# sloup/hessgpu

Hardware: AMD Instinct MI355X
Metric: Mpixels/s end-to-end (pyramid->descriptor), 1920x1080 (higher is better)
Workload: dtype f32; 1 GPU; 1920x1080 synthetic blobs (tests/fixtures.py), default octaves/DoG levels, top-K=4096 [configs[1]]; pipelined_contexts_per_gpu=6, streams_and_copier_threads_per_node=6, descriptor_order=pixel, distinct_images_per_gpu=8, input=u8 luminance resident in HBM; results delivered to host memory

## Files before the change

hessgpu_amd/csrc/hess_ctx.h:

```cpp
#pragma once
#include <hip/hip_runtime.h>
#include <hsa/hsa.h>
#include <hsa/hsa_ext_amd.h>

#include <algorithm>
#include <atomic>
#include <cmath>
#include <condition_variable>
#include <cstdarg>
#include <cerrno>
#include <chrono>
#include <cstdio>
#include <cstdlib>
#include <cstring>
#include <mutex>
#include <new>
#include <string>
#include <thread>
#include <vector>

#include <fcntl.h>
#include <limits.h>
#include <sys/mman.h>
#include <sys/stat.h>
// ... 112 lines not shown
  int ds = 0;
  int img_w = 0, img_h = 0;
  Geom g;
  Taps taps0;
  bool has_taps0 = false;
  int cap_raw = 0, cap_sel = 0, cap_feat = 0;
  bool use_topk = false, multi = false;
  int dim = 0;
  int found_tasks = 0;
  DevBuf gauss, deth, got, input_f32, upsampled, stage, rowoff, level_count, raw_total, found, task_count, raw, sel,
      sel_total, recs, ocount, foffset, fsrc, feat_total, feat_first, img_base, keys, desc;
  DevBuf zeroed;
  size_t zeroed_used = 0;
  bool zero_filled = false;
  struct View { void* p = nullptr; } rowmask, rowcnt, overflow, hist, tk,
      found_count, place_ticket, place_flag;
  int batch = 0;
  int pyramid_batch = 0;
  std::vector<int> counts;
  std::vector<size_t> offs;
  DevBuf h_keys, h_desc, h_small;
  std::string share;
  struct ShareDir {
    uint32_t magic, gen_keys, gen_desc, pad;
    uint64_t keys_bytes, desc_bytes;
    char keys_path[1024], desc_path[1024];
  }* share_dir = nullptr;
  bool share_by_need = false;
  DevBuf h_stage;
  double stamp_submit0 = 0.0, stamp_submit1 = 0.0;
  bool level0_in_lds = false;
// ... 102 lines not shown
```

hessgpu_amd/csrc/hess_dev.h:

```cpp
#pragma once
#include <hip/hip_runtime.h>
#include <stdint.h>

namespace hess {

constexpr int kMaxOct = 16;
constexpr int kMaxDog = 10;
constexpr int kMaxLev = kMaxDog + 3;
constexpr int kMaxTaps = 33;
#ifndef HESS_STREAM_NC
#define HESS_STREAM_NC 2
#endif
constexpr int kStreamCols = HESS_STREAM_NC;
constexpr int kStreamPitch = 62 * kStreamCols;
#ifndef HESS_STREAM_ROWS
#define HESS_STREAM_ROWS 24
#endif
constexpr int kStreamRows = HESS_STREAM_ROWS;
constexpr int kHistBins = 32768;

typedef float hess_v4f __attribute__((ext_vector_type(4)));
__device__ __forceinline__ void store_stream_f4(float* p, float x, float y, float z, float w) {
#ifdef HESS_NO_STREAM_STORES
  *reinterpret_cast<float4*>(p) = make_float4(x, y, z, w);
#else
  __builtin_nontemporal_store((hess_v4f){x, y, z, w}, reinterpret_cast<hess_v4f*>(p));
#endif
}

// ... 151 lines not shown
void launch_dog_planes(hipStream_t st, const Geom& g, const float* gauss, float* deth, int level_max, int batch);
void launch_hessian_level(hipStream_t st, const Geom& g, const float* gauss, float* deth, int level, float norm,
                          int batch, void* zero = nullptr, size_t zero_bytes = 0);

constexpr int kDetectSlots = 64;
struct DetectStore {
  RawKey* found;
  long long stride;
  int ntask;
  int* task_count;
  int* spill_count;
  int cap_spill;
  unsigned* hist;
};
int extrema_tasks(const Geom& g);
void launch_extrema_mark(hipStream_t st, const Geom& g, const DetectParams& dp, const float* gauss,
                         const float* deth, uint64_t* rowmask, int* rowcnt, const DetectStore& ds, int batch,
                         bool dog_mode = false);
bool extrema_streams(const Geom& g);
void launch_extrema_place(hipStream_t st, const Geom& g, const LimitParams& lp, const DetectStore& ds, const uint64_t* rowmask,
                          const int* rowcnt, int* rowoff, int* level_count, int* raw_total, int* overflow, int* ticket,
                          int* flag, RawKey* raw, int cap_raw, int batch);

void launch_topk(hipStream_t st, const Geom& g, int K, const RawKey* raw, const int* raw_total,
                 int cap_raw, unsigned* hist, RawKey* sel, int* sel_total, int cap_sel, int batch, void* scratch,
                 int* overflow);
size_t topk_scratch_bytes(int cap_raw, int batch, int nlev);

void launch_orientation(hipStream_t st, const Geom& g, const OrientParams& op, const RawKey* list,
                        const int* list_total, int cap_list, const float* got, FRec* recs,
                        int* ocount, int batch);
void launch_feature_scan(hipStream_t st, const Geom& g, const LimitParams& lp, int multi, const RawKey* list,
                         const int* list_total, int cap_list, const int* ocount, int* foffset, int* fsrc,
                         int* feat_total, int* feat_first, int cap_feat, int* overflow, int* img_base, int* host_small,
                         int batch);
void launch_descriptor(hipStream_t st, const Geom& g, const DescParams& dp, const RawKey* list,
                       int cap_list, const FRec* recs, const int* fsrc, const int* feat_total,
// ... 6 lines not shown
```

hessgpu_amd/csrc/hess_plan.hip:

```cpp
#include "hess_ctx.h"

namespace hess {

void set_err(hess_ctx* c, const char* fmt, ...) {
  char buf[512];
  va_list ap;
  va_start(ap, fmt);
  vsnprintf(buf, sizeof(buf), fmt, ap);
  va_end(ap);
  try { c->err = buf; } catch (...) {}
  if (c->p.verbose & 1) fprintf(stderr, "hessgpu: %s\n", buf);
}


int ensure(hess_ctx* c, DevBuf& b, size_t bytes, bool pinned_host) {
  if (bytes <= b.bytes) return 0;
  if (pinned_host && c->share_dir && (&b == &c->h_keys || &b == &c->h_desc)) return ensure_shared(c, b, bytes, &b == &c->h_keys ? 'k' : 'd');
  const size_t want = bytes + bytes / 8;
  void* np = nullptr;
  if (pinned_host) HIP_TRY(c, hipHostMalloc(&np, want, hipHostMallocDefault));
  else HIP_TRY(c, hipMalloc(&np, want));
  if (b.p) { if (pinned_host) (void)hipHostFree(b.p); else (void)hipFree(b.p); }
  b.p = np;
  b.bytes = want;
// ... 197 lines not shown
    if (cap_sel < need) cap_sel = need;
    if (cap_feat < need) cap_feat = need;
  }

  int rc;
  if ((rc = ensure(c, c->gauss, (size_t)lvl * 4))) return rc;
  if ((rc = ensure(c, c->deth, (size_t)lvl * 4))) return rc;
  if ((rc = ensure(c, c->got, (size_t)gt * 8))) return rc;
  {
    const int up = ds < 0 ? -ds : 0;
    if ((rc = ensure(c, c->input_f32, (size_t)B * (ws >> up) * (hs >> up) * 4))) return rc;
  }
  if (ds < 0 && (rc = ensure(c, c->upsampled, (size_t)B * ws * hs * 4))) return rc;
  {
    auto up = [](size_t v) { return (v + 255) & ~(size_t)255; };
    const size_t o_found = 256, o_cnt = o_found + up((size_t)3 * B * 4), o_hist = o_cnt + up((size_t)B * g.NR * 4);
    const size_t o_mask = o_hist + (c->use_topk ? up((size_t)B * kHistBins * 4) : 0);
    const size_t o_tk = o_mask + up((size_t)B * g.NM * 8);
    c->zeroed_used = o_tk + (c->use_topk ? up(topk_scratch_bytes(cap_raw, B, g.nlev)) : 0);
    if ((rc = ensure(c, c->zeroed, c->zeroed_used))) return rc;
    char* z = (char*)c->zeroed.p;
    c->overflow.p = z; c->rowcnt.p = z + o_cnt; c->hist.p = z + o_hist; c->rowmask.p = z + o_mask; c->tk.p = z + o_tk;
    c->found_count.p = z + o_found; c->place_ticket.p = z + o_found + (size_t)B * 4; c->place_flag.p = z + o_found + (size_t)2 * B * 4;
  }
  if ((rc = ensure(c, c->rowoff, (size_t)B * g.NR * 4))) return rc;
  if ((rc = ensure(c, c->level_count, (size_t)B * g.nlev * 4))) return rc;
  if ((rc = ensure(c, c->raw_total, (size_t)B * 4))) return rc;
  if ((rc = ensure(c, c->sel_total, (size_t)B * 4))) return rc;
  if ((rc = ensure(c, c->feat_total, (size_t)B * 4))) return rc;
  if ((rc = ensure(c, c->feat_first, (size_t)B * 4))) return rc;
  if ((rc = ensure(c, c->img_base, (size_t)(B + 1) * 4))) return rc;
  if ((rc = ensure(c, c->raw, (size_t)B * cap_raw * sizeof(RawKey)))) return rc;
  {
    int ntask = extrema_tasks(g);
    for (int rows : {kStreamRows / policy::kLatencyStreamRowsDiv, c->stream_rows}) {
      if (rows <= 0) continue;
      Geom gr = g;
      set_stream_rows(gr, rows);
// ... 54 lines not shown
```

hessgpu_amd/csrc/hess_planes.h:

```cpp
#pragma once
#include "hess_dev.h"
#include "hess_devmath.h"

namespace hess {
namespace {

__device__ __forceinline__ float tex1(const float* p, int n, int i) { return (i < 0 || i >= n) ? 0.0f : p[i]; }

__device__ __forceinline__ float lane_prev(float v) {
  return __int_as_float(__builtin_amdgcn_update_dpp(0, __float_as_int(v), 0x138 , 0xf, 0xf, false));
}
__device__ __forceinline__ float lane_next(float v) {
  return __int_as_float(__builtin_amdgcn_update_dpp(0, __float_as_int(v), 0x130 , 0xf, 0xf, false));
}

__device__ __forceinline__ void hessian_rows_body(const float* src, float* dh, float2* gt, int wa, int h, float norm,
                                                  int gid) {
  const int groups_per_row = wa >> 2;
  const int nthreads = groups_per_row * h;
  if (gid >= nthreads) return;
  int row = (int)(((float)gid + 0.5f) * (1.0f / (float)groups_per_row));
  int rem = gid - row * groups_per_row;
  if (rem < 0) { row--; rem += groups_per_row; }
  else if (rem >= groups_per_row) { row++; rem -= groups_per_row; }
  const int x = rem << 2;
  const int n = wa * h;
  const int idx = row * wa + x;

// ... 65 lines not shown
```

hessgpu_amd/csrc/hess_schedule.hip:

```cpp
#include <optional>

#include "hess_ctx.h"

namespace hess {

hipEvent_t get_event(hess_ctx* c) {
  if (!c->pool.empty()) { hipEvent_t e = c->pool.back(); c->pool.pop_back(); return e; }
  hipEvent_t e = nullptr;
  if (hipEventCreate(&e) != hipSuccess) { set_err(c, "hipEventCreate failed: profiling disabled"); c->prof = false; return nullptr; }
  return e;
}
struct ProfScope {
  hess_ctx* c;
  EventPair ep;
  bool on;
  ProfScope(hess_ctx* ctx, int kernel, double bytes, int kernel2 = -1, double in_lds = 0.0) : c(ctx), on(ctx->prof) {
    if (!on) return;
    ep.a = get_event(c); ep.b = get_event(c); ep.kernel = kernel; ep.bytes = bytes; ep.kernel2 = kernel2; ep.in_lds = in_lds;
    if (!ep.a || !ep.b) {
      if (ep.a) c->pool.push_back(ep.a);
      if (ep.b) c->pool.push_back(ep.b);
      on = false;
      return;
    }
// ... 274 lines not shown
  if (!c->zero_filled)
    HIP_TRY(c, hipMemsetAsync(c->zeroed.p, 0, c->zeroed_used, st));
  DetectStore dstore;
  dstore.found = (RawKey*)c->found.p;
  dstore.ntask = extrema_tasks(gx);
  dstore.stride = (long long)c->found_tasks * kDetectSlots + c->cap_raw;
  dstore.task_count = (int*)c->task_count.p;
  dstore.spill_count = (int*)c->found_count.p;
  dstore.cap_spill = c->cap_raw;
  dstore.hist = c->use_topk ? (unsigned*)c->hist.p : nullptr;
  if (dstore.ntask > c->found_tasks) { set_err(c, "detection store laid out for %d scan tasks, the batch has %d", c->found_tasks, dstore.ntask); return HESS_ERR_ARG; }
  {
    double det_bytes = 0;
    for (int o = 0; o < g.noct; o++) det_bytes += 4.0 * s.level_num * g.o[o].plane;
    ProfScope ps(c, HESS_K_EXTREMA, det_bytes * batch);
    launch_extrema_mark(st, gx, dp, gauss, deth, (uint64_t*)c->rowmask.p, (int*)c->rowcnt.p, dstore, batch,
                        s.detector == HESS_DETECTOR_DOG);
  }
  if (c->stage_events) HIP_TRY(c, hipEventRecord(c->ev[2], st));
  {
    ProfScope ps(c, HESS_K_EXTREMA, 0.0);
    launch_extrema_place(st, g, lp, dstore, (const uint64_t*)c->rowmask.p, (const int*)c->rowcnt.p, (int*)c->rowoff.p,
                         (int*)c->level_count.p, (int*)c->raw_total.p, (int*)c->overflow.p, (int*)c->place_ticket.p,
                         (int*)c->place_flag.p, (RawKey*)c->raw.p, c->cap_raw, batch);
  }
  if (c->stage_events) HIP_TRY(c, hipEventRecord(c->ev[3], st));
  const RawKey* list = (const RawKey*)c->raw.p;
  const int* list_total = (const int*)c->raw_total.p;
  int cap_list = c->cap_raw;
  if (c->use_topk) {
    ProfScope ps(c, HESS_K_TOPK, 0.0);
    launch_topk(st, g, p.feature_count_threshold, (const RawKey*)c->raw.p, (const int*)c->raw_total.p, c->cap_raw,
                (unsigned*)c->hist.p, (RawKey*)c->sel.p, (int*)c->sel_total.p, c->cap_sel, batch, c->tk.p, (int*)c->overflow.p);
    list = (const RawKey*)c->sel.p;
    list_total = (const int*)c->sel_total.p;
    cap_list = c->cap_sel;
  }
  c->d_list = list;
  c->d_list_total = list_total;
// ... 189 lines not shown
```

hessgpu_amd/csrc/k_detect.hip:

```cpp
#include <algorithm>
#include <cstddef>
#include <cstdlib>

#include "hess_dev.h"
#include "hess_devmath.h"
#include "hess_planes.h"

namespace hess {

namespace {


struct HessArgs {
  const float* gauss;
  float* deth;
  float2* got;
  int wa, h, plane, B, dog, level_first, batch;
  float inv_groups;
  long long lvl_off, got_off;
  float norm[kMaxLev];
};

__global__ __launch_bounds__(256) void hessian_kernel(HessArgs a) {
  const int z = blockIdx.y;
// ... 256 lines not shown
  int ri = wave - t.b * g.NR;
  int o = 0;
  for (int k = 1; k < g.noct; k++)
    if (g.o[k].row_base <= ri) o = k;
  t.o = o;
  int rel = ri - g.o[o].row_base;
  int lm1 = rel / g.o[o].h;
  t.l = lm1 + 1;
  t.row = rel - lm1 * g.o[o].h;
  t.li = o * g.dog + lm1;
  return t;
}

constexpr int EX_TR = 4, EX_TC = 128, EX_STRIDE = EX_TC + 8 + 4;

template <bool DM>
__global__ __launch_bounds__(256) void extrema_mark_kernel(Geom g, DetectParams dp, const float* gauss, const float* deth,
                                                           uint64_t* rowmask, int* rowcnt, DetectStore ds) {
  extern __shared__ __attribute__((aligned(16))) float tile[];
  __shared__ int nfound;
  __shared__ unsigned short cand[EX_TR * EX_TC];
  __shared__ int ncand;
  const int b = blockIdx.y;
  int o = 0;
  for (int k = 1; k < g.noct; k++)
    if (g.o[k].tile_base <= (int)blockIdx.x) o = k;
  const OctGeom& og = g.o[o];
  const int trel = blockIdx.x - og.tile_base;
  const int ty = trel / og.tiles_x, tx = trel - ty * og.tiles_x;
  const int x0 = tx * EX_TC, y0 = ty * EX_TR;
  const int nlv = g.dog + 2;
  constexpr int ROWS = EX_TR + 2, NG = (EX_TC + 8) / 4;
  const int ngroups = nlv * ROWS * NG;
// ... 77 lines not shown
      KeyVal kv;
      const bool ok = i < nc && key_eval<false, DM>(C, P, N, G, EX_STRIDE, (rl_ + 1) * EX_STRIDE + (cl + 4), dp, &kv,
                                                (long long)row * og.wa + col);
      const uint64_t m = __builtin_amdgcn_ballot_w64(ok);
      int before = 0;
      if (m) {
        if (lane == __builtin_ctzll(m)) before = atomicAdd(&nfound, __popcll(m));
        before = __shfl(before, __builtin_ctzll(m));
      }
      post_detections(sk, before, ok, m, kv, o * g.dog + (l - 1), row, col,
                      og.mask_base + ((l - 1) * og.h + row) * og.w64 + (col >> 6), og.row_base + (l - 1) * og.h + row);
    }
  }
  __syncthreads();
  if (threadIdx.x == 0) ds.task_count[(long long)b * ds.ntask + blockIdx.x] = min(nfound, DT_SLOTS);
}

constexpr int SX_PITCH = kStreamPitch, SX_QCAP = 128;

__device__ __forceinline__ float max3f(float a, float b, float c) { return fmaxf(fmaxf(a, b), c); }
__device__ __forceinline__ float min3f(float a, float b, float c) { return fminf(fminf(a, b), c); }

template <int DOG, bool DM = false>
__global__ __launch_bounds__(256) void extrema_stream_kernel(Geom g, DetectParams dp, const float* gauss, const float* deth,
                                                             unsigned long long* rowmask, int* rowcnt, DetectStore ds) {
  constexpr int NLV = DOG;
  constexpr int NC = kStreamCols;
  __shared__ uint32_t queue[4][SX_QCAP];
  const int lane = threadIdx.x & 63, wv = threadIdx.x >> 6;
  const int b = blockIdx.y;
  const int blk = (int)blockIdx.x;
  int o = 0;
  for (int k = 1; k < g.noct; k++)
    if (g.o[k].stream_base <= blk) o = k;
  const OctGeom& og = g.o[o];
  const int task = (blk - og.stream_base) * 4 + wv;
  const int seg = task / og.strips, strip = task - seg * og.strips;
  const int ys = seg * g.stream_rows;
  int* const my_count = ds.task_count + (long long)b * ds.ntask + blk * 4 + wv;
  if (ys >= og.h) {
    if (lane == 0) *my_count = 0;
    return;
  }
  const int ye = min(ys + g.stream_rows, og.h);
  const int cx = strip * SX_PITCH - NC + NC * lane;
  const bool col_in = cx >= 0 && cx < og.wa;
  const int wa = og.wa, h = og.h;
  const long long lstep = (long long)g.B * og.plane;
  const float* base = deth + og.lvl_off + (long long)b * og.plane + (DM ? lstep : 0);
  const float* sbase = base + lstep;
  const bool own = lane >= 1 && lane <= 62;
  bool cv[NC];
#pragma unroll
  for (int c = 0; c < NC; c++) cv[c] = own && cx + c > 0 && cx + c < wa - 1;
  uint32_t* q = queue[wv];
  int qn = 0;

  struct Row { float v[NC]; };
  auto load_row = [&](int yy, Row (&dst)[NLV]) {
    const int yc = yy < 0 ? 0 : (yy >= h ? h - 1 : yy);
    const long long off = (long long)yc * wa + (col_in ? cx : 0);
#pragma unroll
    for (int l = 0; l < NLV; l++) {
      if (NC == 2) {
        const float2 t = *reinterpret_cast<const float2*>(sbase + l * lstep + off);
        dst[l].v[0] = t.x; dst[l].v[NC - 1] = t.y;
      } else {
#pragma unroll
        for (int c = 0; c < NC; c++) dst[l].v[c] = sbase[l * lstep + off + c];
      }
    }
  };
  const long long fbase = (long long)b * ds.stride;
  const DetectSink sk{ds.found + fbase + (long long)(blk * 4 + wv) * DT_SLOTS, ds.found + fbase + (long long)ds.ntask * DT_SLOTS,
                      ds.spill_count + b, ds.cap_spill, rowmask + (long long)b * g.NM, rowcnt + (long long)b * g.NR,
                      ds.hist ? ds.hist + (long long)b * kHistBins : nullptr};
// ... 3 lines not shown
    const int l = e >> 28, row = (e >> 14) & 0x3FFF, col = e & 0x3FFF;
    const float* C = base + l * lstep;
    KeyVal kv;
    const bool ok = active && key_eval<false, DM>(C, C - lstep, C + lstep, gbase + l * lstep, wa, row * wa + col, dp, &kv);
    const uint64_t m = __builtin_amdgcn_ballot_w64(ok);
    post_detections(sk, nfound, ok, m, kv, o * g.dog + (l - 1), row, col, og.mask_base + ((l - 1) * h + row) * og.w64 + (col >> 6),
                    og.row_base + (l - 1) * h + row);
    nfound += __popcll(m);
  };

  float hmx[NLV][3][NC], hmn[NLV][3][NC];
  float rc[DOG][3][NC];
  auto ingest = [&](const Row (&cur)[NLV], int slot) {
#pragma unroll
    for (int l = 0; l < NLV; l++) {
      const float L = lane_prev(cur[l].v[NC - 1]), R = lane_next(cur[l].v[0]);
#pragma unroll
      for (int c = 0; c < NC; c++) {
        const float left = c == 0 ? L : cur[l].v[c > 0 ? c - 1 : 0];
        const float right = c == NC - 1 ? R : cur[l].v[c < NC - 1 ? c + 1 : c];
        const float a = cur[l].v[c];
        hmx[l][slot][c] = max3f(left, a, right);
        hmn[l][slot][c] = min3f(left, a, right);
        rc[l][slot][c] = a;
      }
    }
  };

  Row cur[NLV], nxt[NLV];
  load_row(ys - 1, cur);
  load_row(ys, nxt);
  ingest(cur, 0);
#pragma unroll
  for (int l = 0; l < NLV; l++) cur[l] = nxt[l];
  load_row(ys + 1, nxt);
  ingest(cur, 1);

  for (int y0 = ys; y0 < ye; y0 += 3) {
#pragma unroll
    for (int s = 0; s < 3; s++) {
      const int y = y0 + s;
      if (y < ye) {
        constexpr int kRing[5] = {0, 1, 2, 0, 1};
        const int sa = kRing[s], sc = kRing[s + 1], sb = kRing[s + 2];
#pragma unroll
        for (int l = 0; l < NLV; l++) cur[l] = nxt[l];
        if (y + 2 <= ye) load_row(y + 2, nxt);
        ingest(cur, sb);
        if (y > 0 && y < h - 1) {
          float m9x[NLV][NC], m9n[NLV][NC];
#pragma unroll
          for (int l = 0; l < NLV; l++)
#pragma unroll
            for (int c = 0; c < NC; c++) {
              m9x[l][c] = max3f(hmx[l][sa][c], hmx[l][sc][c], hmx[l][sb][c]);
              m9n[l][c] = min3f(hmn[l][sa][c], hmn[l][sc][c], hmn[l][sb][c]);
            }
          uint32_t cand = 0;
#pragma unroll
          for (int li = 0; li < DOG; li++)
#pragma unroll
            for (int c = 0; c < NC; c++) {
              const int lo = li > 0 ? li - 1 : li, hi = li < DOG - 1 ? li + 1 : li;
// ... 18 lines not shown
              process(head, true);
              qn -= 64;
              if (lane < qn) q[lane] = tail;
              __builtin_amdgcn_wave_barrier();
            }
          }
        }
      }
    }
  }
  __builtin_amdgcn_wave_barrier();
  if (qn > 0) process(q[lane < qn ? lane : 0], lane < qn);
  if (lane == 0) *my_count = min(nfound, DT_SLOTS);
}

__device__ int apply_level_limits(int* lc, int nlev, const LimitParams& lp, bool generation_stage);


__device__ __forceinline__ void block_scan2(int a, int b, int* ea, int* eb, int* ta, int* tb, int* lds ) {
  const int lane = threadIdx.x & 63, wv = threadIdx.x >> 6;
  int ia = a, ib = b;
#pragma unroll
  for (int d = 1; d < 64; d <<= 1) {
    int na = __shfl_up(ia, d), nb = __shfl_up(ib, d);
    if (lane >= d) { ia += na; ib += nb; }
  }
  __syncthreads();
  if (lane == 63) { lds[wv] = ia; lds[16 + wv] = ib; }
  __syncthreads();
  int oa = 0, ob = 0, sa = 0, sb = 0;
  for (int k = 0; k < 16; k++) {
    if (k < wv) { oa += lds[k]; ob += lds[16 + k]; }
    sa += lds[k]; sb += lds[16 + k];
  }
  *ea = oa + ia - a; *eb = ob + ib - b; *ta = sa; *tb = sb;
}

__device__ int apply_level_limits(int* lc, int nlev, const LimitParams& lp, bool generation_stage) {
  int total = 0;
  const int thr = lp.threshold;
  if (generation_stage) {
    const bool reverse = (lp.method == 1);
    for (int k = 0; k < nlev; k++) {
      int li = reverse ? nlev - 1 - k : k;
      if ((lp.method == 1 || lp.method == 2) && thr > 0 && total > thr) { lc[li] = 0; continue; }
      total += lc[li];
// ... 3 lines not shown
  }
  if (thr > 0 && lp.method != 3) {
    if (lp.method == 2) {
      int i = 0, nf = 0;
      for (; (nf < thr) && (i < nlev); ++i) nf += lc[i];
      for (; i < nlev; ++i) lc[i] = 0;
      if (nf < total) total = nf;
    } else {
      int i = 0;
      while (i < nlev && (total - lc[i]) > thr) { total -= lc[i]; lc[i++] = 0; }
    }
  }
  return total;
}

__device__ void row_scan_block(const Geom& g, const LimitParams& lp, const int* rowcnt, int* rowoff, int* level_count,
                               int* raw_total, int cap_raw, int* overflow, int b) {
  __shared__ int lc[kMaxOct * kMaxDog];
  __shared__ int keep[kMaxOct * kMaxDog];
  __shared__ int lds[64];
  const int tid = threadIdx.x;
  const int* cnt = rowcnt + (long long)b * g.NR;
  int* off = rowoff + (long long)b * g.NR;
  for (int i = tid; i < g.nlev; i += 1024) lc[i] = 0;
  __syncthreads();
  const int per = (g.NR + 1023) >> 10;
  const int r0 = tid * per, r1 = min(g.NR, r0 + per);
  constexpr int RC = 32;
  __shared__ int oct_h[kMaxOct], oct_base[kMaxOct];
  for (int i = tid; i < g.noct; i += 1024) { oct_h[i] = g.o[i].h; oct_base[i] = g.o[i].row_base; }
  __syncthreads();
  if (per <= RC) {
    int cc[RC];
#pragma unroll
    for (int u = 0; u < RC; u++) cc[u] = (u < per && r0 + u < r1) ? cnt[r0 + u] : 0;
    int o = 0;
    for (int k = 1; k < g.noct; k++) if (oct_base[k] <= r0) o = k;
    const int rel = r0 - oct_base[o];
    const int lm0 = rel / oct_h[o];
    const int li0 = o * g.dog + lm0, left0 = oct_h[o] - (rel - lm0 * oct_h[o]);
    int lis[RC];
    {
      int li = li0, lm = lm0, left = left0, oo = o;
#pragma unroll
      for (int u = 0; u < RC; u++) {
        lis[u] = li;
        if (--left == 0) {
          li++;
          if (++lm == g.dog) { lm = 0; oo++; }
          left = oo < g.noct ? oct_h[oo] : 0x7fffffff;
        }
      }
    }
    {
      int run_level = -1, run = 0;
#pragma unroll
      for (int u = 0; u < RC; u++) {
        if (cc[u]) {
          if (lis[u] != run_level) {
            if (run) atomicAdd(&lc[run_level], run);
            run_level = lis[u]; run = 0;
          }
          run += cc[u];
        }
      }
      if (run) atomicAdd(&lc[run_level], run);
    }
    __syncthreads();
    if (tid == 0) {
      int before[kMaxOct * kMaxDog];
      for (int i = 0; i < g.nlev; i++) before[i] = lc[i];
      int total = apply_level_limits(lc, g.nlev, lp, true);
      for (int i = 0; i < g.nlev; i++) {
        keep[i] = (lc[i] == before[i]);
        level_count[b * g.nlev + i] = lc[i];
      }
      raw_total[b] = total < cap_raw ? total : cap_raw;
      if (total > cap_raw) atomicMax(overflow, total);
    }
    __syncthreads();
    int mine = 0;
#pragma unroll
    for (int u = 0; u < RC; u++) {
      cc[u] = (cc[u] && keep[min(lis[u], g.nlev - 1)]) ? cc[u] : 0;
      mine += cc[u];
    }
    int e, e2, tot, tot2;
    block_scan2(mine, 0, &e, &e2, &tot, &tot2, lds);
#pragma unroll
    for (int u = 0; u < RC; u++) {
      if (u < per && r0 + u < r1) off[r0 + u] = e;
      e += cc[u];
    }
    return;
  }
  auto level_of_row = [&](int i) {
    int o = 0;
    for (int k = 1; k < g.noct; k++) if (oct_base[k] <= i) o = k;
    return o * g.dog + (i - oct_base[o]) / oct_h[o];
  };
  {
    int run_level = -1, run = 0;
    for (int i = r0; i < r1; i++) {
      const int c = cnt[i];
      if (!c) continue;
      const int li = level_of_row(i);
      if (li != run_level) {
        if (run) atomicAdd(&lc[run_level], run);
        run_level = li; run = 0;
      }
      run += c;
    }
    if (run) atomicAdd(&lc[run_level], run);
  }
  __syncthreads();
  if (tid == 0) {
    int before[kMaxOct * kMaxDog];
    for (int i = 0; i < g.nlev; i++) before[i] = lc[i];
    int total = apply_level_limits(lc, g.nlev, lp, true);
    for (int i = 0; i < g.nlev; i++) {
      keep[i] = (lc[i] == before[i]);
      level_count[b * g.nlev + i] = lc[i];
    }
    raw_total[b] = total < cap_raw ? total : cap_raw;
    if (total > cap_raw) atomicMax(overflow, total);
  }
  __syncthreads();
  int mine = 0;
  for (int i = r0; i < r1; i++) {
    const int c = cnt[i];
    if (c && keep[level_of_row(i)]) mine += c;
  }
  int e, e2, tot, tot2;
  block_scan2(mine, 0, &e, &e2, &tot, &tot2, lds);
  for (int i = r0; i < r1; i++) {
    off[i] = e;
    const int c = cnt[i];
    if (c && keep[level_of_row(i)]) e += c;
  }
}

constexpr int PL_SPIN_LIMIT = 1 << 21;
#ifndef HESS_PL_PER
#define HESS_PL_PER 2
#endif
constexpr int PL_PER = HESS_PL_PER;
constexpr int PL_CHUNK = 1024 * PL_PER;

__global__ __launch_bounds__(1024) void extrema_place_kernel(Geom g, LimitParams lp, DetectStore ds, const uint64_t* rowmask,
                                                             const int* rowcnt, int* rowoff, int* level_count, int* raw_total,
                                                             int* overflow, int* ticket, int* flag, RawKey* raw, int cap_raw) {
  __shared__ int s_ck;
  const int b = blockIdx.y, tid = threadIdx.x;
  if (tid == 0) s_ck = atomicAdd(&ticket[b], 1);
  __syncthreads();
  const int ck = s_ck;
  const int nslot = ds.ntask * DT_SLOTS;
  const int total = nslot + min(ds.spill_count[b], ds.cap_spill);
  if (ck != 0 && ck * PL_CHUNK >= total) return;
  if (ck == 0) {
    row_scan_block(g, lp, rowcnt, rowoff, level_count, raw_total, cap_raw, overflow, b);
    __threadfence();
    __syncthreads();
    if (tid == 0) __hip_atomic_store(&flag[b], 1, __ATOMIC_RELEASE, __HIP_MEMORY_SCOPE_AGENT);
  }
  struct Pending { uint4 ra, rb; int li, ri, rank; bool valid; };
  auto fetch = [&](int i) {
    Pending p;
    p.valid = i < total && !(i < nslot && (i & (DT_SLOTS - 1)) >= ds.task_count[(long long)b * ds.ntask + i / DT_SLOTS]);
    p.ra = p.rb = make_uint4(0u, 0u, 0u, 0u);
    p.li = p.ri = p.rank = 0;
    if (!p.valid) return p;
    const uint4* const src = reinterpret_cast<const uint4*>(ds.found + (long long)b * ds.stride + i);
    p.ra = src[0]; p.rb = src[1];
    p.li = (int)p.ra.x;
    const int col = (int)p.ra.y, row = (int)p.ra.z;
    const int oct = p.li / g.dog, lm1 = p.li - oct * g.dog;
    const OctGeom& og = g.o[oct];
    p.ri = og.row_base + lm1 * og.h + row;
    const uint64_t* const mrow = rowmask + (long long)b * g.NM + og.mask_base + (lm1 * og.h + row) * og.w64;
    const int wcol = col >> 6;
    p.rank = __popcll(mrow[wcol] & ((1ull << (col & 63)) - 1ull));
    for (int w0 = 0; w0 < wcol; w0 += 8) {
      uint64_t mw[8];
#pragma unroll
      for (int k = 0; k < 8; k++) mw[k] = (w0 + k < wcol) ? mrow[w0 + k] : 0ull;
#pragma unroll
      for (int k = 0; k < 8; k++) p.rank += __popcll(mw[k]);
    }
    return p;
  };
  auto place = [&](const Pending& p) {
    if (!p.valid) return;
    if (__hip_atomic_load(&level_count[b * g.nlev + p.li], __ATOMIC_RELAXED, __HIP_MEMORY_SCOPE_AGENT) == 0) return;
    const int pos = __hip_atomic_load(&rowoff[(long long)b * g.NR + p.ri], __ATOMIC_RELAXED, __HIP_MEMORY_SCOPE_AGENT) + p.rank;
    if (pos < cap_raw) {
      uint4* const dst = reinterpret_cast<uint4*>(raw + (long long)b * cap_raw + pos);
      dst[0] = p.ra;
      dst[1] = p.rb;
    }
  };
  Pending first[PL_PER];
#pragma unroll
  for (int u = 0; u < PL_PER; u++) first[u] = fetch(ck * PL_CHUNK + u * 1024 + tid);
  if (ck != 0) {
    __shared__ int s_ok;
    if (tid == 0) {
      int v = __hip_atomic_load(&flag[b], __ATOMIC_RELAXED, __HIP_MEMORY_SCOPE_AGENT);
      for (int spin = 0; !v && spin < PL_SPIN_LIMIT; spin++) {
        __builtin_amdgcn_s_sleep(32);
        v = __hip_atomic_load(&flag[b], __ATOMIC_RELAXED, __HIP_MEMORY_SCOPE_AGENT);
      }
      if (!v) atomicMax(overflow + 2, 1);
      s_ok = v;
    }
    __syncthreads();
    if (!s_ok) return;
  }
#pragma unroll
  for (int u = 0; u < PL_PER; u++) place(first[u]);
  for (int i0 = (ck + (int)gridDim.x) * PL_CHUNK; i0 < total; i0 += gridDim.x * PL_CHUNK)
    for (int u = 0; u < PL_PER; u++) place(fetch(i0 + u * 1024 + tid));
}


constexpr int TK_PER = 4, TK_CHUNK = 1024 * TK_PER;


__device__ __forceinline__ void topk_find_cut(const unsigned* h, int K, int* lds, int* s_cut, int* s_need) {
  const int tid = threadIdx.x;
  const int owner = 1023 - tid;
  int vals[32];
  {
    const uint4* hv = reinterpret_cast<const uint4*>(h + owner * 32);
#pragma unroll
    for (int q = 0; q < 8; q++) {
      const uint4 v = hv[q];
// ... 168 lines not shown
  hipLaunchKernelGGL(hessian_rows4_kernel, dim3(blocks, batch), dim3(256), 0, st, g, gauss, deth, level, norm,
                     reinterpret_cast<uint4*>(zero), (long long)(zero_bytes / 16));
}

void launch_dog_planes(hipStream_t st, const Geom& g, const float* gauss, float* deth, int level_max, int batch) {
  int blocks = 0;
  for (int o = 0; o < g.noct; o++) blocks += ((g.o[o].plane >> 2) + 255) >> 8;
  hipLaunchKernelGGL(dog_planes_kernel, dim3(blocks, level_max * batch), dim3(256), 0, st, g, gauss, deth, batch);
}

bool extrema_streams(const Geom& g) { return g.dog <= 5 && g.o[0].wa < (1 << 14) && g.o[0].h < (1 << 14); }

int extrema_tasks(const Geom& g) { return extrema_streams(g) ? g.nstream * 4 : g.ntiles; }

void launch_extrema_mark(hipStream_t st, const Geom& g, const DetectParams& dp, const float* gauss,
                         const float* deth, uint64_t* rowmask, int* rowcnt, const DetectStore& ds, int batch, bool dog_mode) {
  if (extrema_streams(g)) {
    unsigned long long* rm = reinterpret_cast<unsigned long long*>(rowmask);
    const dim3 grid(g.nstream, batch), blk(256);
#define HESS_STREAM_LAUNCH(D)                                                                                             \
  do {                                                                                                                    \
    if (dog_mode) hipLaunchKernelGGL((extrema_stream_kernel<D, true>), grid, blk, 0, st, g, dp, gauss, deth, rm, rowcnt, ds); \
    else hipLaunchKernelGGL(extrema_stream_kernel<D>, grid, blk, 0, st, g, dp, gauss, deth, rm, rowcnt, ds);             \
  } while (0)
    switch (g.dog) {
      case 1: HESS_STREAM_LAUNCH(1); break;
      case 2: HESS_STREAM_LAUNCH(2); break;
      case 3: HESS_STREAM_LAUNCH(3); break;
      case 4: HESS_STREAM_LAUNCH(4); break;
      default: HESS_STREAM_LAUNCH(5); break;
    }
#undef HESS_STREAM_LAUNCH
    return;
  }
  const size_t lds = (size_t)(g.dog + 2) * (EX_TR + 2) * EX_STRIDE * sizeof(float);
  static size_t lds_allowed[2] = {0, 0};
  if (lds > lds_allowed[dog_mode]) {
    (void)hipFuncSetAttribute(dog_mode ? reinterpret_cast<const void*>(extrema_mark_kernel<true>)
                                       : reinterpret_cast<const void*>(extrema_mark_kernel<false>),
                              hipFuncAttributeMaxDynamicSharedMemorySize, (int)lds);
    lds_allowed[dog_mode] = lds;
  }
  if (dog_mode)
    hipLaunchKernelGGL(extrema_mark_kernel<true>, dim3(g.ntiles, batch), dim3(256), lds, st, g, dp, gauss, deth, rowmask, rowcnt, ds);
  else
    hipLaunchKernelGGL(extrema_mark_kernel<false>, dim3(g.ntiles, batch), dim3(256), lds, st, g, dp, gauss, deth, rowmask, rowcnt, ds);
}

void launch_extrema_place(hipStream_t st, const Geom& g, const LimitParams& lp, const DetectStore& ds, const uint64_t* rowmask,
                          const int* rowcnt, int* rowoff, int* level_count, int* raw_total, int* overflow, int* ticket,
                          int* flag, RawKey* raw, int cap_raw, int batch) {
  const int chunks = (ds.ntask * DT_SLOTS + std::min(ds.cap_spill, 16 * 1024) + PL_CHUNK - 1) / PL_CHUNK;
  hipLaunchKernelGGL(extrema_place_kernel, dim3(chunks, batch), dim3(1024), 0, st, g, lp, ds, rowmask, rowcnt, rowoff,
                     level_count, raw_total, overflow, ticket, flag, raw, cap_raw);
}

int topk_chunks(int cap_raw) { return (cap_raw + TK_CHUNK - 1) / TK_CHUNK; }

void launch_topk(hipStream_t st, const Geom& g, int K, const RawKey* raw, const int* raw_total, int cap_raw,
                 unsigned* hist, RawKey* sel, int* sel_total, int cap_sel, int batch, void* scratch, int* overflow) {
  const int nchunk = topk_chunks(cap_raw);
  int* ticket = reinterpret_cast<int*>(scratch);
  unsigned long long* state = reinterpret_cast<unsigned long long*>(ticket + ((batch + 1) & ~1));
  int* sel_level_count = reinterpret_cast<int*>(state + (size_t)batch * nchunk);
  hipLaunchKernelGGL(topk_select_kernel, dim3(nchunk, batch), dim3(1024), 0, st, g, K, raw, raw_total, cap_raw, hist,
                     ticket, state, sel, sel_total, sel_level_count, cap_sel, nchunk, overflow);
}

size_t topk_scratch_bytes(int cap_raw, int batch, int nlev) {
// ... 10 lines not shown
```

Before: 23820 Mpix/s.

## Fuse row scan into extrema mark via last-arriving-block, drop place spin-wait

```diff
diff --git a/hessgpu_amd/csrc/hess_ctx.h b/hessgpu_amd/csrc/hess_ctx.h
--- a/hessgpu_amd/csrc/hess_ctx.h
+++ b/hessgpu_amd/csrc/hess_ctx.h
@@ -150,7 +150,7 @@
   size_t zeroed_used = 0;
   bool zero_filled = false;
   struct View { void* p = nullptr; } rowmask, rowcnt, overflow, hist, tk,
-      found_count, place_ticket, place_flag;
+      found_count, scan_arrive;
   int batch = 0;
   int pyramid_batch = 0;
   std::vector<int> counts;
diff --git a/hessgpu_amd/csrc/hess_dev.h b/hessgpu_amd/csrc/hess_dev.h
--- a/hessgpu_amd/csrc/hess_dev.h
+++ b/hessgpu_amd/csrc/hess_dev.h
@@ -12,7 +12,7 @@
 #define HESS_STREAM_NC 2
 #endif
 constexpr int kStreamCols = HESS_STREAM_NC;
-constexpr int kStreamPitch = 62 * kStreamCols;
+constexpr int kStreamPitch = 64 * kStreamCols;
 #ifndef HESS_STREAM_ROWS
 #define HESS_STREAM_ROWS 24
 #endif
@@ -194,13 +194,21 @@
   unsigned* hist;
 };
 int extrema_tasks(const Geom& g);
+struct RowScan {
+  LimitParams lp;
+  int* arrive;
+  int* rowoff;
+  int* level_count;
+  int* raw_total;
+  int* overflow;
+  int cap_raw;
+};
 void launch_extrema_mark(hipStream_t st, const Geom& g, const DetectParams& dp, const float* gauss,
-                         const float* deth, uint64_t* rowmask, int* rowcnt, const DetectStore& ds, int batch,
-                         bool dog_mode = false);
+                         const float* deth, uint64_t* rowmask, int* rowcnt, const DetectStore& ds, const RowScan& rs,
+                         int batch, bool dog_mode = false);
 bool extrema_streams(const Geom& g);
-void launch_extrema_place(hipStream_t st, const Geom& g, const LimitParams& lp, const DetectStore& ds, const uint64_t* rowmask,
-                          const int* rowcnt, int* rowoff, int* level_count, int* raw_total, int* overflow, int* ticket,
-                          int* flag, RawKey* raw, int cap_raw, int batch);
+void launch_extrema_place(hipStream_t st, const Geom& g, const DetectStore& ds, const uint64_t* rowmask, const int* rowoff,
+                          const int* level_count, RawKey* raw, int cap_raw, int batch);
 
 void launch_topk(hipStream_t st, const Geom& g, int K, const RawKey* raw, const int* raw_total,
                  int cap_raw, unsigned* hist, RawKey* sel, int* sel_total, int cap_sel, int batch, void* scratch,
diff --git a/hessgpu_amd/csrc/hess_plan.hip b/hessgpu_amd/csrc/hess_plan.hip
--- a/hessgpu_amd/csrc/hess_plan.hip
+++ b/hessgpu_amd/csrc/hess_plan.hip
@@ -235,14 +235,14 @@
   if (ds < 0 && (rc = ensure(c, c->upsampled, (size_t)B * ws * hs * 4))) return rc;
   {
     auto up = [](size_t v) { return (v + 255) & ~(size_t)255; };
-    const size_t o_found = 256, o_cnt = o_found + up((size_t)3 * B * 4), o_hist = o_cnt + up((size_t)B * g.NR * 4);
+    const size_t o_found = 256, o_cnt = o_found + up((size_t)2 * B * 4), o_hist = o_cnt + up((size_t)B * g.NR * 4);
     const size_t o_mask = o_hist + (c->use_topk ? up((size_t)B * kHistBins * 4) : 0);
     const size_t o_tk = o_mask + up((size_t)B * g.NM * 8);
     c->zeroed_used = o_tk + (c->use_topk ? up(topk_scratch_bytes(cap_raw, B, g.nlev)) : 0);
     if ((rc = ensure(c, c->zeroed, c->zeroed_used))) return rc;
     char* z = (char*)c->zeroed.p;
     c->overflow.p = z; c->rowcnt.p = z + o_cnt; c->hist.p = z + o_hist; c->rowmask.p = z + o_mask; c->tk.p = z + o_tk;
-    c->found_count.p = z + o_found; c->place_ticket.p = z + o_found + (size_t)B * 4; c->place_flag.p = z + o_found + (size_t)2 * B * 4;
+    c->found_count.p = z + o_found; c->scan_arrive.p = z + o_found + (size_t)B * 4;
   }
   if ((rc = ensure(c, c->rowoff, (size_t)B * g.NR * 4))) return rc;
   if ((rc = ensure(c, c->level_count, (size_t)B * g.nlev * 4))) return rc;
diff --git a/hessgpu_amd/csrc/hess_planes.h b/hessgpu_amd/csrc/hess_planes.h
--- a/hessgpu_amd/csrc/hess_planes.h
+++ b/hessgpu_amd/csrc/hess_planes.h
@@ -12,6 +12,12 @@
 }
 __device__ __forceinline__ float lane_next(float v) {
   return __int_as_float(__builtin_amdgcn_update_dpp(0, __float_as_int(v), 0x130 , 0xf, 0xf, false));
+}
+__device__ __forceinline__ float lane_prev_edge(float v, float edge) {
+  return __int_as_float(__builtin_amdgcn_update_dpp(__float_as_int(edge), __float_as_int(v), 0x138 , 0xf, 0xf, false));
+}
+__device__ __forceinline__ float lane_next_edge(float v, float edge) {
+  return __int_as_float(__builtin_amdgcn_update_dpp(__float_as_int(edge), __float_as_int(v), 0x130 , 0xf, 0xf, false));
 }
 
 __device__ __forceinline__ void hessian_rows_body(const float* src, float* dh, float2* gt, int wa, int h, float norm,
diff --git a/hessgpu_amd/csrc/hess_schedule.hip b/hessgpu_amd/csrc/hess_schedule.hip
--- a/hessgpu_amd/csrc/hess_schedule.hip
+++ b/hessgpu_amd/csrc/hess_schedule.hip
@@ -312,15 +312,16 @@
     double det_bytes = 0;
     for (int o = 0; o < g.noct; o++) det_bytes += 4.0 * s.level_num * g.o[o].plane;
     ProfScope ps(c, HESS_K_EXTREMA, det_bytes * batch);
-    launch_extrema_mark(st, gx, dp, gauss, deth, (uint64_t*)c->rowmask.p, (int*)c->rowcnt.p, dstore, batch,
+    const RowScan rscan{lp, (int*)c->scan_arrive.p, (int*)c->rowoff.p, (int*)c->level_count.p, (int*)c->raw_total.p,
+                        (int*)c->overflow.p, c->cap_raw};
+    launch_extrema_mark(st, gx, dp, gauss, deth, (uint64_t*)c->rowmask.p, (int*)c->rowcnt.p, dstore, rscan, batch,
                         s.detector == HESS_DETECTOR_DOG);
   }
   if (c->stage_events) HIP_TRY(c, hipEventRecord(c->ev[2], st));
   {
     ProfScope ps(c, HESS_K_EXTREMA, 0.0);
-    launch_extrema_place(st, g, lp, dstore, (const uint64_t*)c->rowmask.p, (const int*)c->rowcnt.p, (int*)c->rowoff.p,
-                         (int*)c->level_count.p, (int*)c->raw_total.p, (int*)c->overflow.p, (int*)c->place_ticket.p,
-                         (int*)c->place_flag.p, (RawKey*)c->raw.p, c->cap_raw, batch);
+    launch_extrema_place(st, g, dstore, (const uint64_t*)c->rowmask.p, (const int*)c->rowoff.p, (const int*)c->level_count.p,
+                         (RawKey*)c->raw.p, c->cap_raw, batch);
   }
   if (c->stage_events) HIP_TRY(c, hipEventRecord(c->ev[3], st));
   const RawKey* list = (const RawKey*)c->raw.p;
diff --git a/hessgpu_amd/csrc/k_detect.hip b/hessgpu_amd/csrc/k_detect.hip
--- a/hessgpu_amd/csrc/k_detect.hip
+++ b/hessgpu_amd/csrc/k_detect.hip
@@ -294,9 +294,12 @@
 
 constexpr int EX_TR = 4, EX_TC = 128, EX_STRIDE = EX_TC + 8 + 4;
 
+template <int NT>
+__device__ __forceinline__ void scan_arrive(const Geom& g, const RowScan& rs, const int* rowcnt, int b, int nwg);
+
 template <bool DM>
 __global__ __launch_bounds__(256) void extrema_mark_kernel(Geom g, DetectParams dp, const float* gauss, const float* deth,
-                                                           uint64_t* rowmask, int* rowcnt, DetectStore ds) {
+                                                           uint64_t* rowmask, int* rowcnt, DetectStore ds, RowScan rs) {
   extern __shared__ __attribute__((aligned(16))) float tile[];
   __shared__ int nfound;
   __shared__ unsigned short cand[EX_TR * EX_TC];
@@ -404,6 +407,7 @@
   }
   __syncthreads();
   if (threadIdx.x == 0) ds.task_count[(long long)b * ds.ntask + blockIdx.x] = min(nfound, DT_SLOTS);
+  scan_arrive<256>(g, rs, rowcnt, b, g.ntiles);
 }
 
 constexpr int SX_PITCH = kStreamPitch, SX_QCAP = 128;
@@ -411,15 +415,13 @@
 __device__ __forceinline__ float max3f(float a, float b, float c) { return fmaxf(fmaxf(a, b), c); }
 __device__ __forceinline__ float min3f(float a, float b, float c) { return fminf(fminf(a, b), c); }
 
-template <int DOG, bool DM = false>
-__global__ __launch_bounds__(256) void extrema_stream_kernel(Geom g, DetectParams dp, const float* gauss, const float* deth,
-                                                             unsigned long long* rowmask, int* rowcnt, DetectStore ds) {
+template <int DOG, bool DM>
+__device__ __forceinline__ void stream_task(const Geom& g, const DetectParams& dp, const float* gauss, const float* deth,
+                                            unsigned long long* rowmask, int* rowcnt, const DetectStore& ds, uint32_t* q,
+                                            int b, int blk) {
   constexpr int NLV = DOG;
   constexpr int NC = kStreamCols;
-  __shared__ uint32_t queue[4][SX_QCAP];
   const int lane = threadIdx.x & 63, wv = threadIdx.x >> 6;
-  const int b = blockIdx.y;
-  const int blk = (int)blockIdx.x;
   int o = 0;
   for (int k = 1; k < g.noct; k++)
     if (g.o[k].stream_base <= blk) o = k;
@@ -433,23 +435,30 @@
     return;
   }
   const int ye = min(ys + g.stream_rows, og.h);
-  const int cx = strip * SX_PITCH - NC + NC * lane;
-  const bool col_in = cx >= 0 && cx < og.wa;
+  const int cx = strip * SX_PITCH + NC * lane;
+  const bool col_in = cx < og.wa;
   const int wa = og.wa, h = og.h;
+  const bool edge_lane = lane == 0 || lane == 63;
+  const int hx = lane == 0 ? strip * SX_PITCH - 1 : (strip + 1) * SX_PITCH;
+  const int hxc = (hx >= 0 && hx < wa) ? hx : 0;
   const long long lstep = (long long)g.B * og.plane;
   const float* base = deth + og.lvl_off + (long long)b * og.plane + (DM ? lstep : 0);
   const float* sbase = base + lstep;
-  const bool own = lane >= 1 && lane <= 62;
   bool cv[NC];
 #pragma unroll
-  for (int c = 0; c < NC; c++) cv[c] = own && cx + c > 0 && cx + c < wa - 1;
-  uint32_t* q = queue[wv];
+  for (int c = 0; c < NC; c++) cv[c] = cx + c > 0 && cx + c < wa - 1;
   int qn = 0;
 
-  struct Row { float v[NC]; };
+  struct Row { float v[NC]; float e; };
   auto load_row = [&](int yy, Row (&dst)[NLV]) {
     const int yc = yy < 0 ? 0 : (yy >= h ? h - 1 : yy);
     const long long off = (long long)yc * wa + (col_in ? cx : 0);
+#pragma unroll
+    for (int l = 0; l < NLV; l++) dst[l].e = 0.0f;
+    if (edge_lane) {
+#pragma unroll
+      for (int l = 0; l < NLV; l++) dst[l].e = sbase[l * lstep + (long long)yc * wa + hxc];
+    }
 #pragma unroll
     for (int l = 0; l < NLV; l++) {
       if (NC == 2) {
@@ -483,7 +492,7 @@
   auto ingest = [&](const Row (&cur)[NLV], int slot) {
 #pragma unroll
     for (int l = 0; l < NLV; l++) {
-      const float L = lane_prev(cur[l].v[NC - 1]), R = lane_next(cur[l].v[0]);
+      const float L = lane_prev_edge(cur[l].v[NC - 1], cur[l].e), R = lane_next_edge(cur[l].v[0], cur[l].e);
 #pragma unroll
       for (int c = 0; c < NC; c++) {
         const float left = c == 0 ? L : cur[l].v[c > 0 ? c - 1 : 0];
@@ -496,14 +505,15 @@
     }
   };
 
-  Row cur[NLV], nxt[NLV];
-  load_row(ys - 1, cur);
-  load_row(ys, nxt);
-  ingest(cur, 0);
-#pragma unroll
-  for (int l = 0; l < NLV; l++) cur[l] = nxt[l];
+  Row nxt[NLV];
+  {
+    Row first[NLV];
+    load_row(ys - 1, first);
+    load_row(ys, nxt);
+    ingest(first, 0);
+  }
+  ingest(nxt, 1);
   load_row(ys + 1, nxt);
-  ingest(cur, 1);
 
   for (int y0 = ys; y0 < ye; y0 += 3) {
 #pragma unroll
@@ -512,10 +522,8 @@
       if (y < ye) {
         constexpr int kRing[5] = {0, 1, 2, 0, 1};
         const int sa = kRing[s], sc = kRing[s + 1], sb = kRing[s + 2];
-#pragma unroll
-        for (int l = 0; l < NLV; l++) cur[l] = nxt[l];
+        ingest(nxt, sb);
         if (y + 2 <= ye) load_row(y + 2, nxt);
-        ingest(cur, sb);
         if (y > 0 && y < h - 1) {
           float m9x[NLV][NC], m9n[NLV][NC];
 #pragma unroll
@@ -564,9 +572,27 @@
   if (lane == 0) *my_count = min(nfound, DT_SLOTS);
 }
 
+template <int DOG, bool DM = false>
+__global__ __launch_bounds__(256) void extrema_stream_kernel(Geom g, DetectParams dp, const float* gauss, const float* deth,
+                                                             unsigned long long* rowmask, int* rowcnt, DetectStore ds,
+                                                             RowScan rs) {
+  __shared__ uint32_t queue[4][SX_QCAP];
+  const int b = blockIdx.y;
+#ifdef HESS_SCAN_PLAIN_ORDER
+  const int blk = (int)blockIdx.x;
+#else
+  const int per_xcd = (int)gridDim.x >> 3;
+  const int blk = (((int)blockIdx.x + b) & 7) * per_xcd + ((int)blockIdx.x >> 3);
+#endif
+  if (blk >= g.nstream) return;
+  stream_task<DOG, DM>(g, dp, gauss, deth, rowmask, rowcnt, ds, queue[threadIdx.x >> 6], b, blk);
+  scan_arrive<256>(g, rs, rowcnt, b, g.nstream);
+}
+
 __device__ int apply_level_limits(int* lc, int nlev, const LimitParams& lp, bool generation_stage);
 
 
+template <int NW = 16>
 __device__ __forceinline__ void block_scan2(int a, int b, int* ea, int* eb, int* ta, int* tb, int* lds ) {
   const int lane = threadIdx.x & 63, wv = threadIdx.x >> 6;
   int ia = a, ib = b;
@@ -579,7 +605,7 @@
   if (lane == 63) { lds[wv] = ia; lds[16 + wv] = ib; }
   __syncthreads();
   int oa = 0, ob = 0, sa = 0, sb = 0;
-  for (int k = 0; k < 16; k++) {
+  for (int k = 0; k < NW; k++) {
     if (k < wv) { oa += lds[k]; ob += lds[16 + k]; }
     sa += lds[k]; sb += lds[16 + k];
   }
@@ -613,7 +639,10 @@
   return total;
 }
 
-__device__ void row_scan_block(const Geom& g, const LimitParams& lp, const int* rowcnt, int* rowoff, int* level_count,
+__device__ __forceinline__ int rowcount(const int* p) { return __hip_atomic_load(p, __ATOMIC_RELAXED, __HIP_MEMORY_SCOPE_AGENT); }
+
+template <int NT>
+__device__ __forceinline__ void row_scan_block(const Geom& g, const LimitParams& lp, const int* rowcnt, int* rowoff, int* level_count,
                                int* raw_total, int cap_raw, int* overflow, int b) {
   __shared__ int lc[kMaxOct * kMaxDog];
   __shared__ int keep[kMaxOct * kMaxDog];
@@ -621,29 +650,29 @@
   const int tid = threadIdx.x;
   const int* cnt = rowcnt + (long long)b * g.NR;
   int* off = rowoff + (long long)b * g.NR;
-  for (int i = tid; i < g.nlev; i += 1024) lc[i] = 0;
-  __syncthreads();
-  const int per = (g.NR + 1023) >> 10;
+  for (int i = tid; i < g.nlev; i += NT) lc[i] = 0;
+  __syncthreads();
+  const int per = (g.NR + NT - 1) / NT;
   const int r0 = tid * per, r1 = min(g.NR, r0 + per);
   constexpr int RC = 32;
   __shared__ int oct_h[kMaxOct], oct_base[kMaxOct];
-  for (int i = tid; i < g.noct; i += 1024) { oct_h[i] = g.o[i].h; oct_base[i] = g.o[i].row_base; }
-  __syncthreads();
-  if (per <= RC) {
+  for (int i = tid; i < g.noct; i += NT) { oct_h[i] = g.o[i].h; oct_base[i] = g.o[i].row_base; }
+  __syncthreads();
+  constexpr int LS = 16;
+  if (per <= RC && g.o[0].wa < (1 << LS)) {
     int cc[RC];
 #pragma unroll
-    for (int u = 0; u < RC; u++) cc[u] = (u < per && r0 + u < r1) ? cnt[r0 + u] : 0;
+    for (int u = 0; u < RC; u++) cc[u] = (u < per && r0 + u < r1) ? rowcount(cnt + r0 + u) : 0;
     int o = 0;
     for (int k = 1; k < g.noct; k++) if (oct_base[k] <= r0) o = k;
     const int rel = r0 - oct_base[o];
     const int lm0 = rel / oct_h[o];
     const int li0 = o * g.dog + lm0, left0 = oct_h[o] - (rel - lm0 * oct_h[o]);
-    int lis[RC];
     {
       int li = li0, lm = lm0, left = left0, oo = o;
 #pragma unroll
       for (int u = 0; u < RC; u++) {
-        lis[u] = li;
+        cc[u] |= li << LS;
         if (--left == 0) {
           li++;
           if (++lm == g.dog) { lm = 0; oo++; }
@@ -655,23 +684,23 @@
       int run_level = -1, run = 0;
 #pragma unroll
       for (int u = 0; u < RC; u++) {
-        if (cc[u]) {
-          if (lis[u] != run_level) {
+        const int c = cc[u] & ((1 << LS) - 1), l = cc[u] >> LS;
+        if (c) {
+          if (l != run_level) {
             if (run) atomicAdd(&lc[run_level], run);
-            run_level = lis[u]; run = 0;
+            run_level = l; run = 0;
           }
-          run += cc[u];
+          run += c;
         }
       }
       if (run) atomicAdd(&lc[run_level], run);
     }
     __syncthreads();
     if (tid == 0) {
-      int before[kMaxOct * kMaxDog];
-      for (int i = 0; i < g.nlev; i++) before[i] = lc[i];
+      for (int i = 0; i < g.nlev; i++) keep[i] = lc[i];
       int total = apply_level_limits(lc, g.nlev, lp, true);
       for (int i = 0; i < g.nlev; i++) {
-        keep[i] = (lc[i] == before[i]);
+        keep[i] = (lc[i] == keep[i]);
         level_count[b * g.nlev + i] = lc[i];
       }
       raw_total[b] = total < cap_raw ? total : cap_raw;
@@ -681,11 +710,12 @@
     int mine = 0;
 #pragma unroll
     for (int u = 0; u < RC; u++) {
-      cc[u] = (cc[u] && keep[min(lis[u], g.nlev - 1)]) ? cc[u] : 0;
+      const int c = cc[u] & ((1 << LS) - 1);
+      cc[u] = (c && keep[min(cc[u] >> LS, g.nlev - 1)]) ? c : 0;
       mine += cc[u];
     }
     int e, e2, tot, tot2;
-    block_scan2(mine, 0, &e, &e2, &tot, &tot2, lds);
+    block_scan2<NT / 64>(mine, 0, &e, &e2, &tot, &tot2, lds);
 #pragma unroll
     for (int u = 0; u < RC; u++) {
       if (u < per && r0 + u < r1) off[r0 + u] = e;
@@ -701,7 +731,7 @@
   {
     int run_level = -1, run = 0;
     for (int i = r0; i < r1; i++) {
-      const int c = cnt[i];
+      const int c = rowcount(cnt + i);
       if (!c) continue;
       const int li = level_of_row(i);
       if (li != run_level) {
@@ -714,11 +744,10 @@
   }
   __syncthreads();
   if (tid == 0) {
-    int before[kMaxOct * kMaxDog];
-    for (int i = 0; i < g.nlev; i++) before[i] = lc[i];
+    for (int i = 0; i < g.nlev; i++) keep[i] = lc[i];
     int total = apply_level_limits(lc, g.nlev, lp, true);
     for (int i = 0; i < g.nlev; i++) {
-      keep[i] = (lc[i] == before[i]);
+      keep[i] = (lc[i] == keep[i]);
       level_count[b * g.nlev + i] = lc[i];
     }
     raw_total[b] = total < cap_raw ? total : cap_raw;
@@ -727,42 +756,42 @@
   __syncthreads();
   int mine = 0;
   for (int i = r0; i < r1; i++) {
-    const int c = cnt[i];
+    const int c = rowcount(cnt + i);
     if (c && keep[level_of_row(i)]) mine += c;
   }
   int e, e2, tot, tot2;
-  block_scan2(mine, 0, &e, &e2, &tot, &tot2, lds);
+  block_scan2<NT / 64>(mine, 0, &e, &e2, &tot, &tot2, lds);
   for (int i = r0; i < r1; i++) {
     off[i] = e;
-    const int c = cnt[i];
+    const int c = rowcount(cnt + i);
     if (c && keep[level_of_row(i)]) e += c;
   }
 }
 
-constexpr int PL_SPIN_LIMIT = 1 << 21;
+template <int NT>
+__device__ __forceinline__ void scan_arrive(const Geom& g, const RowScan& rs, const int* rowcnt, int b, int nwg) {
+  __shared__ int s_last;
+  __builtin_amdgcn_s_waitcnt(0x0F70);
+  __syncthreads();
+  if (threadIdx.x == 0)
+    s_last = __hip_atomic_fetch_add(&rs.arrive[b], 1, __ATOMIC_RELAXED, __HIP_MEMORY_SCOPE_AGENT) == nwg - 1;
+  __syncthreads();
+  if (!s_last) return;
+  __builtin_amdgcn_fence(__ATOMIC_ACQUIRE, "agent");
+  row_scan_block<NT>(g, rs.lp, rowcnt, rs.rowoff, rs.level_count, rs.raw_total, rs.cap_raw, rs.overflow, b);
+}
+
 #ifndef HESS_PL_PER
 #define HESS_PL_PER 2
 #endif
 constexpr int PL_PER = HESS_PL_PER;
 constexpr int PL_CHUNK = 1024 * PL_PER;
 
-__global__ __launch_bounds__(1024) void extrema_place_kernel(Geom g, LimitParams lp, DetectStore ds, const uint64_t* rowmask,
-                                                             const int* rowcnt, int* rowoff, int* level_count, int* raw_total,
-                                                             int* overflow, int* ticket, int* flag, RawKey* raw, int cap_raw) {
-  __shared__ int s_ck;
+__global__ __launch_bounds__(1024) void extrema_place_kernel(Geom g, DetectStore ds, const uint64_t* rowmask, const int* rowoff,
+                                                             const int* level_count, RawKey* raw, int cap_raw) {
   const int b = blockIdx.y, tid = threadIdx.x;
-  if (tid == 0) s_ck = atomicAdd(&ticket[b], 1);
-  __syncthreads();
-  const int ck = s_ck;
   const int nslot = ds.ntask * DT_SLOTS;
   const int total = nslot + min(ds.spill_count[b], ds.cap_spill);
-  if (ck != 0 && ck * PL_CHUNK >= total) return;
-  if (ck == 0) {
-    row_scan_block(g, lp, rowcnt, rowoff, level_count, raw_total, cap_raw, overflow, b);
-    __threadfence();
-    __syncthreads();
-    if (tid == 0) __hip_atomic_store(&flag[b], 1, __ATOMIC_RELEASE, __HIP_MEMORY_SCOPE_AGENT);
-  }
   struct Pending { uint4 ra, rb; int li, ri, rank; bool valid; };
   auto fetch = [&](int i) {
     Pending p;
@@ -791,35 +820,21 @@
   };
   auto place = [&](const Pending& p) {
     if (!p.valid) return;
-    if (__hip_atomic_load(&level_count[b * g.nlev + p.li], __ATOMIC_RELAXED, __HIP_MEMORY_SCOPE_AGENT) == 0) return;
-    const int pos = __hip_atomic_load(&rowoff[(long long)b * g.NR + p.ri], __ATOMIC_RELAXED, __HIP_MEMORY_SCOPE_AGENT) + p.rank;
+    if (level_count[b * g.nlev + p.li] == 0) return;
+    const int pos = rowoff[(long long)b * g.NR + p.ri] + p.rank;
     if (pos < cap_raw) {
       uint4* const dst = reinterpret_cast<uint4*>(raw + (long long)b * cap_raw + pos);
       dst[0] = p.ra;
       dst[1] = p.rb;
     }
   };
-  Pending first[PL_PER];
-#pragma unroll
-  for (int u = 0; u < PL_PER; u++) first[u] = fetch(ck * PL_CHUNK + u * 1024 + tid);
-  if (ck != 0) {
-    __shared__ int s_ok;
-    if (tid == 0) {
-      int v = __hip_atomic_load(&flag[b], __ATOMIC_RELAXED, __HIP_MEMORY_SCOPE_AGENT);
-      for (int spin = 0; !v && spin < PL_SPIN_LIMIT; spin++) {
-        __builtin_amdgcn_s_sleep(32);
-        v = __hip_atomic_load(&flag[b], __ATOMIC_RELAXED, __HIP_MEMORY_SCOPE_AGENT);
-      }
-      if (!v) atomicMax(overflow + 2, 1);
-      s_ok = v;
-    }
-    __syncthreads();
-    if (!s_ok) return;
-  }
-#pragma unroll
-  for (int u = 0; u < PL_PER; u++) place(first[u]);
-  for (int i0 = (ck + (int)gridDim.x) * PL_CHUNK; i0 < total; i0 += gridDim.x * PL_CHUNK)
-    for (int u = 0; u < PL_PER; u++) place(fetch(i0 + u * 1024 + tid));
+  for (int i0 = (int)blockIdx.x * PL_CHUNK; i0 < total; i0 += gridDim.x * PL_CHUNK) {
+    Pending p[PL_PER];
+#pragma unroll
+    for (int u = 0; u < PL_PER; u++) p[u] = fetch(i0 + u * 1024 + tid);
+#pragma unroll
+    for (int u = 0; u < PL_PER; u++) place(p[u]);
+  }
 }
 
 
@@ -1018,14 +1033,15 @@
 int extrema_tasks(const Geom& g) { return extrema_streams(g) ? g.nstream * 4 : g.ntiles; }
 
 void launch_extrema_mark(hipStream_t st, const Geom& g, const DetectParams& dp, const float* gauss,
-                         const float* deth, uint64_t* rowmask, int* rowcnt, const DetectStore& ds, int batch, bool dog_mode) {
+                         const float* deth, uint64_t* rowmask, int* rowcnt, const DetectStore& ds, const RowScan& rs, int batch,
+                         bool dog_mode) {
   if (extrema_streams(g)) {
     unsigned long long* rm = reinterpret_cast<unsigned long long*>(rowmask);
-    const dim3 grid(g.nstream, batch), blk(256);
+    const dim3 grid(((g.nstream + 7) >> 3) << 3, batch), blk(256);
 #define HESS_STREAM_LAUNCH(D)                                                                                             \
   do {                                                                                                                    \
-    if (dog_mode) hipLaunchKernelGGL((extrema_stream_kernel<D, true>), grid, blk, 0, st, g, dp, gauss, deth, rm, rowcnt, ds); \
-    else hipLaunchKernelGGL(extrema_stream_kernel<D>, grid, blk, 0, st, g, dp, gauss, deth, rm, rowcnt, ds);             \
+    if (dog_mode) hipLaunchKernelGGL((extrema_stream_kernel<D, true>), grid, blk, 0, st, g, dp, gauss, deth, rm, rowcnt, ds, rs); \
+    else hipLaunchKernelGGL(extrema_stream_kernel<D>, grid, blk, 0, st, g, dp, gauss, deth, rm, rowcnt, ds, rs);             \
   } while (0)
     switch (g.dog) {
       case 1: HESS_STREAM_LAUNCH(1); break;
@@ -1046,17 +1062,16 @@
     lds_allowed[dog_mode] = lds;
   }
   if (dog_mode)
-    hipLaunchKernelGGL(extrema_mark_kernel<true>, dim3(g.ntiles, batch), dim3(256), lds, st, g, dp, gauss, deth, rowmask, rowcnt, ds);
+    hipLaunchKernelGGL(extrema_mark_kernel<true>, dim3(g.ntiles, batch), dim3(256), lds, st, g, dp, gauss, deth, rowmask, rowcnt, ds, rs);
   else
-    hipLaunchKernelGGL(extrema_mark_kernel<false>, dim3(g.ntiles, batch), dim3(256), lds, st, g, dp, gauss, deth, rowmask, rowcnt, ds);
-}
-
-void launch_extrema_place(hipStream_t st, const Geom& g, const LimitParams& lp, const DetectStore& ds, const uint64_t* rowmask,
-                          const int* rowcnt, int* rowoff, int* level_count, int* raw_total, int* overflow, int* ticket,
-                          int* flag, RawKey* raw, int cap_raw, int batch) {
+    hipLaunchKernelGGL(extrema_mark_kernel<false>, dim3(g.ntiles, batch), dim3(256), lds, st, g, dp, gauss, deth, rowmask, rowcnt, ds, rs);
+}
+
+void launch_extrema_place(hipStream_t st, const Geom& g, const DetectStore& ds, const uint64_t* rowmask, const int* rowoff,
+                          const int* level_count, RawKey* raw, int cap_raw, int batch) {
   const int chunks = (ds.ntask * DT_SLOTS + std::min(ds.cap_spill, 16 * 1024) + PL_CHUNK - 1) / PL_CHUNK;
-  hipLaunchKernelGGL(extrema_place_kernel, dim3(chunks, batch), dim3(1024), 0, st, g, lp, ds, rowmask, rowcnt, rowoff,
-                     level_count, raw_total, overflow, ticket, flag, raw, cap_raw);
+  hipLaunchKernelGGL(extrema_place_kernel, dim3(chunks, batch), dim3(1024), 0, st, g, ds, rowmask, rowoff, level_count, raw,
+                     cap_raw);
 }
 
 int topk_chunks(int cap_raw) { return (cap_raw + TK_CHUNK - 1) / TK_CHUNK; }
```

Measured after the change: 24360 Mpix/s (median of 6 runs). 1.02x the previous value.
